# lyd405121/ti-raytrace

Measured on AMD Instinct MI355X. Metric: Mrays/s (primary+secondary) at 1024² 100k-tri, 1/2/4/8 GPU + HBM GB/s, higher is better.
Workload: dtype f32

## Files before the change

ti_raytrace_amd/_native.py:

```python
import ctypes as C
import os

import numpy as np

_HERE = os.path.dirname(os.path.abspath(__file__))
LIB_PATH = os.environ.get("TIRT_LIB_PATH") or os.path.join(_HERE, "csrc", "libtirt.so")

_f32p = np.ctypeslib.ndpointer(dtype=np.float32, flags="C_CONTIGUOUS")
_i32p = np.ctypeslib.ndpointer(dtype=np.int32, flags="C_CONTIGUOUS")


class TirtError(RuntimeError):
    pass


class TirtStackOverflow(TirtError):

    def __init__(self, msg, stats):
        TirtError.__init__(self, msg)
        self.stats = stats


ERR_STACK = -4

# ... 22 lines not shown
DEBUG_GNORMAL = 3

AOV_WORDS = 8
AOV_ALBEDO = 0
AOV_NORMAL = 3
AOV_DEPTH = 6
AOV_ALPHA = 7

MOM_WORDS = 8
MOM_N = 0
MOM_MEAN = 1
MOM_M2 = 4
MOM_BAD = 7

MOTION_WORDS = 8

SF_GLASS, SF_ENV, SF_LIGHT_TRI, SF_LIGHT_SPOT_LASER, SF_NO_LIGHT, SF_LIGHT_SPHERE, SF_LIGHT_OTHER = 1, 2, 4, 8, 16, 32, 64
SF_ALL = 127
SF_TEXTURE = 128
SHADE_INSTANTIATIONS = (SF_LIGHT_SPHERE, SF_LIGHT_TRI, SF_ALL, SF_ALL | SF_TEXTURE)
SF_TEXTURE_PARAM = 256
SHADE_INSTANTIATION_MAPS = SF_ALL | SF_TEXTURE | SF_TEXTURE_PARAM
SF_CUTOUT = 512
SF_ENV_SAMPLE = 1024
SHADE_INSTANTIATIONS_ENV = (SF_ALL | SF_ENV_SAMPLE, SHADE_INSTANTIATION_MAPS | SF_ENV_SAMPLE)
KAT_ENV_SAMPLE_IN, KAT_ENV_SAMPLE_OUT = 2, 10
KAT_ENV_PDF_IN, KAT_ENV_PDF_OUT = 3, 5
KAT_ALPHA_IN, KAT_ALPHA_OUT = 3, 2
KAT_MAPS_IN, KAT_MAPS_OUT = 3, 8
KAT_STEP_IN, KAT_STEP_OUT = 23, 28

OPTIONS = {
    "shade_specialize": (1, "1: the narrowest instantiation of k_shade / k_shade_spec that covers the scene's feature word; 0: the generic kernel"),
}

_vp = C.c_void_p
SIGNATURES = {
    "tirt_last_error": (C.c_char_p, []),
    "tirt_version": (C.c_int, []),
    "tirt_device_count": (C.c_int, [C.POINTER(C.c_int)]),
    "tirt_create": (C.c_int, [C.c_int, C.POINTER(_vp)]),
    "tirt_destroy": (None, [_vp]),
    "tirt_sync": (C.c_int, [_vp]),
    "tirt_set_option": (C.c_int, [_vp, C.c_char_p, C.c_double]),
    "tirt_scene_upload": (C.c_int, [_vp, _f32p, C.c_int, _i32p, C.c_int, _f32p, C.c_int,
                                    _f32p, C.c_int, _i32p, C.c_int, C.c_int, _f32p, _f32p]),
    "tirt_material_upload": (C.c_int, [_vp, _f32p, C.c_int]),
    "tirt_env_upload": (C.c_int, [_vp, _i32p, C.c_int, C.c_int, C.c_float]),
    "tirt_texture_upload": (C.c_int, [_vp, C.c_int, _vp, C.c_int64, _vp, _vp, _vp, _vp]),
    "tirt_kat_texture": (C.c_int, [_vp, _f32p, C.c_int, _f32p, C.c_int, C.c_int]),
    "tirt_kat_material_maps": (C.c_int, [_vp, _f32p, C.c_int, _f32p, C.c_int, C.c_int]),
    "tirt_texture_cutout": (C.c_int, [_vp, _vp, C.c_int]),
    "tirt_kat_texture_alpha": (C.c_int, [_vp, _f32p, C.c_int, _f32p, C.c_int, C.c_int]),
    "tirt_shade_features": (C.c_int, [_vp, C.POINTER(C.c_uint32)]),
    "tirt_shade_features_host": (C.c_int, [_f32p, C.c_int, _i32p, C.c_int, _f32p, C.c_int, _i32p, C.c_int, _vp, C.c_int, C.c_int, C.c_float,
                                           C.POINTER(C.c_uint32)]),
    "tirt_shade_features_host_env": (C.c_int, [_f32p, C.c_int, _i32p, C.c_int, _f32p, C.c_int, _i32p, C.c_int, _vp, C.c_int, C.c_int, C.c_float,
                                               C.c_int, C.POINTER(C.c_uint32)]),
    "tirt_env_sampling": (C.c_int, [_vp, C.c_int, C.c_float]),
    "tirt_env_table_download": (C.c_int, [_vp, _vp, _vp, _vp, C.POINTER(C.c_int32)]),
    "tirt_kat_env_sample": (C.c_int, [_vp, _f32p, C.c_int, _f32p, C.c_int, C.c_int]),
    "tirt_kat_env_pdf": (C.c_int, [_vp, _f32p, C.c_int, _f32p, C.c_int, C.c_int]),
    "tirt_lbvh_build": (C.c_int, [_vp]),
    "tirt_lbvh_download": (C.c_int, [_vp, _vp, _vp, _vp]),
    "tirt_traversal_tree_download": (C.c_int, [_vp, _vp]),
    "tirt_wide_tree_download": (C.c_int, [_vp, _vp, _vp, _vp, _vp, _vp, _vp]),
# ... 733 lines not shown
```

ti_raytrace_amd/csrc/tirt_api.hip:

```cpp
#include "tirt_internal.h"
#include "tirt_spectral.h"
#include <stddef.h>
#include <algorithm>
#include <mutex>
#include <string.h>

namespace tirt {

static thread_local std::string g_error;
void set_error(const std::string &msg) { g_error = msg; }

SceneView scene_view(const tirt_ctx *c)
{
    SceneView s;
    s.vertex = c->vertex.as<float>(); s.primitive = c->primitive.as<int>(); s.material = c->material.as<float>();
    s.shape = c->shape.as<float>(); s.light = c->light.as<int>(); s.env = c->env.as<int>();
    s.mat_lrgb = c->mat_lrgb.as<float>(); s.shade_rec = c->shade_rec.as<float4>(); s.light_rec = c->light_rec.as<float4>();
    s.tex = c->tex_count > 0 ? c->tex.as<int>() : nullptr;
    s.n = c->n; s.light_count = c->light_count; s.env_w = c->env_w; s.env_h = c->env_h; s.env_power = c->env_power;
    return s;
}
BvhView bvh_view(const tirt_ctx *c)
{
    BvhView b;
// ... 452 lines not shown
    if (!strcmp(name, "plan_batches")) { TIRT_REQUIRE(value >= 0.0 && value <= 64.0, "plan_batches: 0 (automatic) .. 64"); if (flush_pending(c)) return TIRT_ERR_HIP; c->plan_nb = (int)value; return TIRT_OK; }
    if (!strcmp(name, "plan_lanes")) { TIRT_REQUIRE(value >= 0.0 && value <= TIRT_MAX_LANES, "plan_lanes: 0 (automatic) .. the lane count"); if (flush_pending(c)) return TIRT_ERR_HIP; c->plan_lanes = (int)value; return TIRT_OK; }
    if (!strcmp(name, "job_frames")) { TIRT_REQUIRE(value >= 0.0 && value <= 1.0e9, "job_frames out of range"); c->job_frames = (long)value; return TIRT_OK; }
    if (!strcmp(name, "merge_paths")) { TIRT_REQUIRE(value >= 0.0 && value <= 1.0e9, "merge_paths out of range"); c->merge_paths = (size_t)value; c->merge_user = true; return TIRT_OK; }
    if (!strcmp(name, "batch_paths")) {
        TIRT_REQUIRE(value >= 1.0 && value <= 1.0e9, "tirt_set_option: batch_paths out of range");
        c->batch_paths = (size_t)value; c->batch_user = true; return TIRT_OK;
    }
    if (!strcmp(name, "trace_lds_depth")) {
        TIRT_REQUIRE(value >= 12 && value <= 64, "trace_lds_depth: 12..64");
        TIRT_REQUIRE(trace_lds_bytes((int)value) <= c->lds_optin, "trace_lds_depth: stacks + tree top exceed the LDS a block can have on this device");
        c->tr_lds_depth = (int)value; return TIRT_OK;
    }
    if (!strcmp(name, "bdpt_stack_size")) { TIRT_REQUIRE(value >= 16 && value <= 4096, "bdpt_stack_size: 16..4096"); c->bdpt_stack = (int)value; return TIRT_OK; }
    if (!strcmp(name, "trace_timeline")) { c->timeline_arm = (int)value; c->timeline_waves = 0; return TIRT_OK; }
    if (!strcmp(name, "trace_refill_min")) { TIRT_REQUIRE(value >= 1 && value <= 64, "trace_refill_min: 1..64"); c->tr_refill_min = (int)value; return TIRT_OK; }
    if (!strcmp(name, "trace_node_min")) { TIRT_REQUIRE(value >= 1 && value <= 64, "trace_node_min: 1..64"); c->tr_node_min = (int)value; return TIRT_OK; }
    if (!strcmp(name, "bdpt_bounded")) { c->bdpt_bounded = value != 0.0 ? 1 : 0; return TIRT_OK; }
    if (!strcmp(name, "bdpt_state_fill")) { TIRT_REQUIRE(value == 0.0 || value == 1.0 || value == 2.0, "bdpt_state_fill: 0 (none), 1 (zeros) or 2 (poison)"); c->bdpt_state_fill = (int)value; return TIRT_OK; }
    if (!strcmp(name, "primary_beams")) { TIRT_REQUIRE(value == 0.0 || value == 1.0, "primary_beams: 0 or 1"); if (flush_pending(c)) return TIRT_ERR_HIP; c->primary_beams = (int)value; return TIRT_OK; }
    if (!strcmp(name, "primary_beams_rebuild")) { if (flush_pending(c)) return TIRT_ERR_HIP; c->pvb_valid = false; return TIRT_OK; }
    if (!strcmp(name, "primary_beams_diag")) { if (flush_pending(c)) return TIRT_ERR_HIP; c->pvb_diag = value != 0.0; return TIRT_OK; }
    if (!strcmp(name, "primary_beams_min_frames")) { TIRT_REQUIRE(value >= 1.0 && value <= 1.0e6, "primary_beams_min_frames out of range"); if (flush_pending(c)) return TIRT_ERR_HIP; c->primary_beams_min_frames = (int)value; return TIRT_OK; }
    if (!strcmp(name, "bdpt_lanes")) { TIRT_REQUIRE(value >= 1.0 && value <= 4.0, "bdpt_lanes: 1..4"); if (sync_all(c)) return TIRT_ERR_HIP; c->bdpt_lanes = (int)value; return TIRT_OK; }
    if (!strcmp(name, "bdpt_batch_items")) { TIRT_REQUIRE(value >= 1.0 && value <= 1.0e9, "bdpt_batch_items out of range"); c->bdpt_batch_items = (size_t)value; return TIRT_OK; }
    if (!strcmp(name, "bdpt_mem_budget")) { TIRT_REQUIRE(value >= 0, "bdpt_mem_budget: bytes >= 0"); c->bdpt_mem_budget = (size_t)value; return TIRT_OK; }
    if (!strcmp(name, "trace_slices")) {
        const int iv = (int)value;
        TIRT_REQUIRE(iv >= 1 && iv <= 64 && (iv & (iv - 1)) == 0, "trace_slices: power of two, 1..64");
        int l = 0; while ((1 << l) < iv) l++;
        c->tr_slice_log2 = l; return TIRT_OK;
    }
    if (!strcmp(name, "shade_specialize")) { TIRT_REQUIRE(value == 0.0 || value == 1.0, "shade_specialize: 0 (generic kernel) or 1"); if (flush_pending(c)) return TIRT_ERR_HIP; c->shade_specialize = (int)value; return TIRT_OK; }
    if (!strcmp(name, "shade_grid")) { TIRT_REQUIRE(value >= 1 && value <= 65536, "shade_grid: 1..65536"); c->sh_grid = (int)value; c->grid_user = true; return TIRT_OK; }
    if (!strcmp(name, "path_order_blocks")) { c->path_order_blocks = value != 0.0; return TIRT_OK; }
    if (!strcmp(name, "slices_contiguous")) { c->slices_contiguous = value != 0.0; return TIRT_OK; }
    if (!strcmp(name, "trace_grid_alone")) { TIRT_REQUIRE(value >= 1 && value <= 16384, "trace_grid_alone: 1..16384"); c->tr_grid_alone = (int)value; return TIRT_OK; }
    if (!strcmp(name, "query_chunk_rays")) {
        TIRT_REQUIRE(value >= 256.0 && value <= (double)(1 << 27), "query_chunk_rays: 256 .. 2^27");
        c->query_chunk = (size_t)value; return TIRT_OK;
    }
    if (!strcmp(name, "trace_grid")) { TIRT_REQUIRE(value >= 1 && value <= 16384, "trace_grid: 1..16384"); c->tr_grid = (int)value; c->grid_user = true; return TIRT_OK; }
    set_error(std::string("tirt_set_option: unknown option ") + name);
    return TIRT_ERR_ARG;
}

int tirt_scene_upload(tirt_ctx *c, const float *vertex, int nv, const int32_t *primitive, int n, const float *material, int nm,
                      const float *shape, int ns, const int32_t *light, int nl, int light_count, const float bmin[3], const float bmax[3])
{
    CTX(c);
    if (sync_all(c)) return TIRT_ERR_HIP;
    TIRT_REQUIRE(n >= 1 && nv >= 0 && nm >= 1 && ns >= 1 && nl >= 1, "tirt_scene_upload: need n,nm,ns,nl >= 1");
    TIRT_REQUIRE(vertex && primitive && material && shape && light && bmin && bmax, "tirt_scene_upload: null pointer");
    TIRT_REQUIRE(light_count >= 0 && light_count <= nl, "tirt_scene_upload: light_count out of range");
    TIRT_REQUIRE((long long)2 * n - 1 < (1ll << 24), "tirt_scene_upload: node indices are stored as f32 (exact below 2^24 nodes)");
    for (int i = 0; i < n; i++) {
        const int32_t *pr = primitive + (size_t)i * 3;
        if (pr[0] == PRIMITIVE_TRI) { TIRT_REQUIRE(pr[1] >= 0 && pr[1] + 2 < nv, "tirt_scene_upload: vertex index out of range"); }
        else { TIRT_REQUIRE(pr[1] >= 0 && pr[1] < ns, "tirt_scene_upload: shape index out of range"); }
        TIRT_REQUIRE(pr[2] >= 0 && pr[2] < nm, "tirt_scene_upload: material index out of range");
    }
    for (int i = 0; i < nl; i++) TIRT_REQUIRE(light[i] >= 0 && light[i] < n, "tirt_scene_upload: light index out of range");
    if (int rc = check_material_textures("tirt_scene_upload", material, nm, c->tex_count)) return rc;
    c->sphere_prims.clear(); c->sphere_geom.clear();
    c->h_mat_on_tri.assign((size_t)nm, 0);
    for (int i = 0; i < n; i++) {
// ... 684 lines not shown
        (void)hipEventRecord(c->ev1, c->stream);
        e = hipEventSynchronize(c->ev1);
        float ms = 0.0f;
        if (e == hipSuccess) e = hipEventElapsedTime(&ms, c->ev0, c->ev1);
        if (rep > 0 && ms < best) best = ms;
    }
    rec.release(); out.release();
    TIRT_HIP(e);
    *gbps_out = (double)blocks * 256.0 * (double)iters * 64.0 / ((double)best * 1.0e-3) / 1.0e9;
    return TIRT_OK;
}

int tirt_stats(tirt_ctx *c, tirt_stats_t *out)
{
    CTX(c);
    TIRT_REQUIRE(out, "tirt_stats: null");
    if (ensure_counters(c)) return TIRT_ERR_HIP;
    DevCounters h;
    if (sync_all(c)) return TIRT_ERR_HIP;
    TIRT_HIP(hipMemcpyAsync(&h, c->dev_counters.p, sizeof(h), hipMemcpyDeviceToHost, c->stream));
    TIRT_HIP(hipStreamSynchronize(c->stream));
    drain_render_events(c);
    out->rays_closest = h.rays_closest; out->rays_shadow = h.rays_shadow;
    out->box_closest = h.box_closest; out->leaf_closest = h.leaf_closest;
    out->box_shadow = h.box_shadow; out->leaf_shadow = h.leaf_shadow;
    out->shaded = h.shaded; out->paths = h.paths; out->stack_overflow = h.stack_overflow;
    out->diag_it_node = h.it_node; out->diag_lanes_node = h.lanes_node; out->diag_it_leaf = h.it_leaf;
    out->diag_lanes_leaf = h.lanes_leaf; out->diag_refills = h.refills; out->diag_it_outer = h.it_outer;
    out->diag_wave_ticks = h.wave_ticks; out->diag_drain_ticks = h.drain_ticks; out->diag_waves = h.waves;
    out->ms_build = c->ms_build; out->ms_render = c->ms_render;
    out->ms_trace_closest = c->ms_trace_closest; out->ms_trace_shadow = c->ms_trace_shadow; out->ms_shade = c->ms_shade;
    out->launches_trace_closest = c->launches_trace_closest; out->launches_trace_shadow = c->launches_trace_shadow;
    out->launches_shade = c->launches_shade; out->launches_tail = 0;
    if (h.stack_overflow > 0) {
        set_error("traversal stack overflow on " + std::to_string((unsigned long long)h.stack_overflow) + " rays: raise stack_size");
        TIRT_HIP(hipMemsetAsync((char *)c->dev_counters.p + offsetof(DevCounters, stack_overflow), 0, sizeof(h.stack_overflow), c->stream));
        TIRT_HIP(hipStreamSynchronize(c->stream));
        return TIRT_ERR_STACK;
    }
    return TIRT_OK;
}

static void drain_pvb_events(tirt_ctx *c)
{
    for (auto &pr : c->pvb_ev) {
        float ms = 0.0f;
        if (hipEventElapsedTime(&ms, pr.first, pr.second) == hipSuccess) c->pvb_build_ns += (unsigned long long)((double)ms * 1.0e6);
        (void)hipEventDestroy(pr.first); (void)hipEventDestroy(pr.second);
    }
    c->pvb_ev.clear();
    (void)hipGetLastError();
}

int tirt_primary_beam_stats(tirt_ctx *c, uint64_t out[12])
{
    TIRT_REQUIRE(c && out, "tirt_primary_beam_stats: null arguments");
    for (int k = 0; k < 12; k++) out[k] = 0;
    if (sync_all(c)) return TIRT_ERR_HIP;
    drain_pvb_events(c);
    out[5] = c->pvb_builds; out[6] = c->pvb_build_ns; out[7] = c->pvb_skipped;
    if (!c->pvb_stat.p) return TIRT_OK;
    unsigned long long h[12];
    TIRT_HIP(hipMemcpy(h, c->pvb_stat.p, sizeof(h), hipMemcpyDeviceToHost));
    for (int k = 0; k < 5; k++) out[k] = h[k];
    for (int k = 8; k < 12; k++) out[k] = h[k];
    return TIRT_OK;
// ... 43 lines not shown
```

ti_raytrace_amd/csrc/tirt_internal.h:

```cpp
#pragma once
#include <hip/hip_runtime.h>
#include <stdint.h>
#include <stdio.h>
#include <initializer_list>
#include <string>
#include <type_traits>
#include <vector>
#include "../../include/tirt.h"
#include "tirt_device.h"

namespace tirt {

void set_error(const std::string &msg);

#define TIRT_HIP(call)                                                                          \
    do {                                                                                        \
        hipError_t e__ = (call);                                                                \
        if (e__ != hipSuccess) {                                                                \
            tirt::set_error(std::string(#call) + ": " + hipGetErrorString(e__));                \
            return TIRT_ERR_HIP;                                                                \
        }                                                                                       \
    } while (0)

#define TIRT_REQUIRE(cond, msg)                                                                 \
// ... 139 lines not shown
    float *sdist;
    int *sdst;
    float *fr, *fg, *fb;
    float *scw, *fw;
};

struct TileMap { int tile_rank, tile_count, tile_size, H, blocked, F; const int *pixels; };
TD void slot_to_frame_pixel(const TileMap &m, int P, int slot, int &f, int &k)
{
    if (m.F > 0) { const int c = slot >> 6, kb = c / m.F; f = c - kb * m.F; k = (kb << 6) | (slot & 63); }
    else { f = slot / P; k = slot - f * P; }
}
TD int frame_pixel_to_slot(const TileMap &m, int P, int f, int k)
{ return m.F > 0 ? ((((k >> 6) * m.F + f) << 6) | (k & 63)) : f * P + k; }
TD int local_to_pixel(const TileMap &m, int k)
{
    int lt = k / m.tile_size, within = k - lt * m.tile_size;
    if (m.blocked) {
        const int rows = m.H >> 3;
        const int b = within >> 6, l = within & 63;
        const int bc = b / rows, bj = b - bc * rows;
        within = ((bc << 3) + (l >> 3)) * m.H + (bj << 3) + (l & 7);
    }
    return (lt * m.tile_count + m.tile_rank) * m.tile_size + within;
}

template <bool LIST> TD int mapped_pixel(const TileMap &m, int k) { if constexpr (LIST) return m.pixels[k]; else return local_to_pixel(m, k); }

struct DevCounters {
    unsigned long long rays_closest, rays_shadow, box_closest, leaf_closest, box_shadow, leaf_shadow;
    unsigned long long shaded, paths, stack_overflow;
    unsigned long long it_node, lanes_node, it_leaf, lanes_leaf, refills, it_outer;
    unsigned long long wave_ticks, drain_ticks, waves;
};

#define TIRT_MAX_LANES 8
struct Lane {
    hipStream_t stream = nullptr;
    hipEvent_t film_done = nullptr; bool film_recorded = false;
    hipEvent_t aov_done = nullptr;
    size_t path_capacity = 0;
    DevBuf path_mem, counters_mem, spill;
    PathState ps;
};

}

struct tirt_ctx {
    int device = 0;
    hipStream_t stream = nullptr;
    hipEvent_t ev0 = nullptr, ev1 = nullptr;

    int nv = 0, n = 0, nm = 0, ns = 0, nl = 0, light_count = 0;
    float bmin[3] = {0, 0, 0}, bmax[3] = {0, 0, 0};
    tirt::DevBuf vertex, primitive, material, shape, light, env, mat_lrgb, shade_rec, light_rec;
    bool shade_rec_valid = false;
    bool light_rec_valid = false;
    int env_w = 0, env_h = 0; float env_power = 0.0f;
    std::vector<int> tex_cutout; std::vector<unsigned char> h_mat_on_tri; bool has_cutout = false;
    tirt::DevBuf cut_uv, cut_flags; bool cut_rec_valid = false, cut_tagged = false;
    tirt::DevBuf tex; int tex_count = 0;
    std::vector<float> h_material; std::vector<int> h_light_kind; bool env_lit = false;
    unsigned shade_features = 127u;
    int env_sample_on = 0; float env_share = 0.5f; bool env_tab_valid = false;
    int shade_specialize = 1;

    bool built = false;
    tirt::DevBuf morton_unsorted;
    tirt::DevBuf keys_a, keys_b, vals_a, vals_b;
    tirt::DevBuf hist;
    tirt::DevBuf morton_sorted;
    tirt::DevBuf bvh_node, compact;
    tirt::DevBuf parent, flag, subtree, build_status, leaf_compact;
    tirt::DevBuf wnode, tri, prim_slot;
    tirt::DevBuf cnode, cparent, csize, wide_queue, wide_levels;
    int wide_nodes = 0;
    tirt::DevBuf sah_compact, sah_csize, sah_parent, wide_dp, sah_box, sah_idx, sah_tasks, sah_counts;
    int use_sah = 1, sah_levels = 0, built_sah = 0;
    std::vector<int> sphere_prims;
    std::vector<float> sphere_geom;
    tirt::DevBuf timeline; int timeline_arm = -1, timeline_waves = 0;
    int n_far_nodes = 0;
    int wide_dp_on = 0;
    float grid_min[3] = {0, 0, 0}, grid_cell[3] = {1, 1, 1}, grid_inv_cell[3] = {1, 1, 1}, grid_inv_extent[3] = {1, 1, 1};
    size_t lds_optin = 65536;
    float root_min[3], root_max[3]; int root_code = 0;
    float wide_pad = 0.0f; int shapes_boxed = 0;

    tirt::CameraView cam; float view[16]; bool cam_set = false;

    int W = 0, H = 0, tile_rank = 0, tile_count = 1, tile_size = 4096, tile_blocked = 0;
    long npix_local = 0;
    tirt::DevBuf hdr, rgb;
    tirt::DevBuf aov;
    hipEvent_t last_aov = nullptr;
    tirt::DevBuf mom, mom_cnt;
    tirt::DevBuf pixset, pixset_tmp; long pixset_n = -1;
    tirt::DevBuf tp_mem; int tp_cur = 0; bool tp_valid = false; tirt_temporal_camera_t tp_cam = {};
// ... 193 lines not shown
```

ti_raytrace_amd/csrc/tirt_render.hip:

```cpp
#include "tirt_internal.h"
#include "tirt_spectral.h"

namespace tirt {

constexpr int TR_GRID_MAX = 2048;

enum { KIND_CLOSEST = 0, KIND_SHADOW_ACC = 1, KIND_MIXED = 2, KIND_QUERY = 3 };
#if !defined(TIRT_EXPERIMENTS) && (defined(TR_PAD) || defined(TR_PADG))
#error "the bound ladder (TR_PAD / TR_PADG) needs an experiments build: add -DTIRT_EXPERIMENTS"
#endif
struct TraceArgs {
    BvhView bvh;
    const float *ox, *oy, *oz, *dx, *dy, *dz;
    float eye[3];
    const int *count_ptr; int count_fixed;
    float4 *hit;
    const int *sprim, *sdst; const float *sdist, *scr, *scg, *scb; float *rr, *rg, *rb, *fr, *fg, *fb;
    const float *scw; float *rw, *fw;
    int *spill; int spill_depth;
    const float *sox, *soy, *soz, *sdx, *sdy, *sdz; const int *scount_ptr;
    int *fetch; int slice_log2;
    int slices_contig;
    int lds_depth;
    int refill_min;
    int node_min;
    DevCounters *ctr; int2 *per_ray_counts;
    unsigned long long *timeline;
    int no_ray_count;
    const float4 *ray4;
    const int *ray_index;
};
struct TraceArgsCut : TraceArgs { CutView cut; };
template <bool CUTOUT> struct trace_args_of { typedef TraceArgs type; };
template <> struct trace_args_of<true> { typedef TraceArgsCut type; };

struct ShadeStep {
    bool want_next = false, want_shadow = false, shaded = false;
    v3 next_o = V(0.0f, 0.0f, 0.0f), next_d = next_o, next_thr = next_o, sh_o = next_o, sh_d = next_o, sh_c = next_o;
    float next_pdf = 0.0f, sh_dist = 0.0f; int next_spec = 0, sh_expect = -2;
};
template <unsigned FEAT, bool LIST = false>
TD void shade_path(const SceneView &sc, const TileMap &tm, int P, uint32_t frame_begin, uint32_t seed, int bounce, int last_bounce, int slot,
                   const v3 origin, const v3 direction, const float4 hrec, v3 throughout, v3 &radiance, float brdf_pdf, int perfect_spec, ShadeStep &s)
{
    int f, k; slot_to_frame_pixel(tm, P, slot, f, k);
    const uint32_t pixel = (uint32_t)mapped_pixel<LIST>(tm, k);
    const uint32_t frame = frame_begin + (uint32_t)f;
    const uint32_t dim0 = TM_DIM_BOUNCE0 + TM_DIMS_PER_BOUNCE * (uint32_t)bounce;
    const float t = hrec.x;
    constexpr bool ENV_NEE = (FEAT & SF_ENV_SAMPLE) != 0u;
    [[maybe_unused]] float p_env = 0.0f;
    if constexpr (ENV_NEE) p_env = sc.light_count == 0 ? 1.0f : env_table(sc).share;
    if (t < INF_VALUE) {
        const int prim_id = __float_as_int(hrec.w);
        int mat_id;
        const HitAttr h = hit_attributes_rec<(FEAT & (SF_TEXTURE | SF_TEXTURE_PARAM)) != 0u>(sc.shade_rec, origin, direction, prim_id, t, hrec.y, hrec.z, mat_id);
        v3 normal = h.nor;
        if constexpr ((FEAT & SF_TEXTURE_PARAM) != 0u) {
            const int nor_id = material_map(sc.material + (size_t)mat_id * MAT_VEC, 9);
            if (nor_id >= 0) normal = tex_normal_rec(sc.tex, sc.shade_rec, nor_id, prim_id, h.tex, normal);
        }
        const v3 fnormal = normal * signf(dot(-direction, h.gnor));
        const float *m = sc.material + (size_t)mat_id * MAT_VEC;
        const v3 mat_color = V(m[2], m[3], m[4]);
// ... 519 lines not shown
        }

        const bool from_pend = STASH && pend != 0;
        const bool leaf_now = have && (from_pend || (cur < 0 && cur != TR_SENT));
        if (COUNT) {
            const int n_l = __popcll(ballot64(leaf_now));
            if (n_l) { d_it_leaf++; d_lanes_leaf += (unsigned long long)n_l; }
        }
        if (leaf_now) {
            const int code = ~(from_pend ? pend : cur);
            if (COUNT) nleaf += 1;
            bool accepted;
            if constexpr (CUTOUT) accepted = trace_leaf_step<MODE != TIRT_TRAVERSE_EXHAUSTIVE, true, CutSource>(b, r, par, code, hit_t, hit_u, hit_v, hit_prim, hit_leaf);
            else accepted = trace_leaf_step<MODE != TIRT_TRAVERSE_EXHAUSTIVE>(b, r, par, code, hit_t, hit_u, hit_v, hit_prim, hit_leaf);
            if (from_pend) pend = 0; else TR_POP(cur);
            if (accepted) {
                lim = __builtin_fminf(__builtin_fminf(cull_far < 0.0f ? INF_VALUE : hit_t * 1.0001f, __builtin_fabsf(cull_far)), INF_VALUE);
                if (BOUNDED && hit_prim != expect && hit_t < settle) { cur = TR_SENT; paged = 0; pend = 0; }
            }
        }

        if (ballot64(have && cur == TR_SENT && paged > 0) != 0ull) {
            if (have && cur == TR_SENT && paged > 0) { TR_PAGE_IN(); TR_POP(cur); }
        }

        if (have && cur == TR_SENT && pend == 0) {
            TR_COLD(ca);
            float4 *const c_hit = ca->hit;
            const int *const c_sdst = MAY_SHADOW ? ca->sdst : nullptr;
            float *const c_rr = MAY_SHADOW ? ca->rr : nullptr, *const c_rg = MAY_SHADOW ? ca->rg : nullptr, *const c_rb = MAY_SHADOW ? ca->rb : nullptr;
            float *const c_fr = MAY_SHADOW ? ca->fr : nullptr, *const c_fg = MAY_SHADOW ? ca->fg : nullptr, *const c_fb = MAY_SHADOW ? ca->fb : nullptr;
            const float *const c_scr = MAY_SHADOW ? ca->scr : nullptr, *const c_scg = MAY_SHADOW ? ca->scg : nullptr, *const c_scb = MAY_SHADOW ? ca->scb : nullptr;
            const float *const c_scw = MAY_SHADOW ? ca->scw : nullptr;
            if (MAY_SHADOW) asm volatile("" :: "s"(c_hit), "s"(c_sdst), "s"(c_rr), "s"(c_rg), "s"(c_rb), "s"(c_fr), "s"(c_fg), "s"(c_fb), "s"(c_scr), "s"(c_scg), "s"(c_scb), "s"(c_scw));
            if (!(MAY_SHADOW && is_sh) || KIND == KIND_QUERY) {
                { typedef float f4n __attribute__((ext_vector_type(4))); f4n hv__ = {hit_t, hit_u, hit_v, __int_as_float(hit_prim)}; __builtin_nontemporal_store(hv__, (f4n *)&c_hit[q]); }
            } else if (hit_prim == expect) {
                const int dst = TR_LDS_(c_sdst[q]);
                float *pr = dst >= 0 ? c_rr + dst : c_fr + ~dst;
                float *pg = dst >= 0 ? c_rg + dst : c_fg + ~dst;
                float *pb = dst >= 0 ? c_rb + dst : c_fb + ~dst;
                *pr = *pr + TR_LDS_(c_scr[q]); *pg = *pg + TR_LDS_(c_scg[q]); *pb = *pb + TR_LDS_(c_scb[q]);
                if (c_scw) { float *pw = dst >= 0 ? ca->rw + dst : ca->fw + ~dst; *pw = *pw + c_scw[q]; }
            }
            if (COUNT) {
                if (MAY_SHADOW && is_sh) { sum_box_s += nbox; sum_leaf_s += nleaf; }
                else { sum_box += nbox; sum_leaf += nleaf; }
                if (ca->per_ray_counts) ca->per_ray_counts[q] = make_int2((int)nbox, (int)nleaf);
            }
            if (n_overflow) n_over++;
            have = false; sa = sa_bottom;
        }
    }
    TR_COLD(ca);
    if (ca->ctr) {
        if (COUNT) {
            sum_box = wave_sum(sum_box); sum_leaf = wave_sum(sum_leaf);
            sum_box_s = wave_sum(sum_box_s); sum_leaf_s = wave_sum(sum_leaf_s);
            if (lane == 0 && (sum_box | sum_leaf)) { atomicAdd(&ca->ctr->box_closest, sum_box); atomicAdd(&ca->ctr->leaf_closest, sum_leaf); }
            if (lane == 0 && (sum_box_s | sum_leaf_s)) { atomicAdd(&ca->ctr->box_shadow, sum_box_s); atomicAdd(&ca->ctr->leaf_shadow, sum_leaf_s); }
        }
        if (COUNT) { d_outer = wave_sum(d_outer); if (lane == 0) atomicAdd(&ca->ctr->it_outer, d_outer); }
        if (COUNT && lane == 0) {
            atomicAdd(&ca->ctr->it_node, d_it_node); atomicAdd(&ca->ctr->lanes_node, d_lanes_node);
            atomicAdd(&ca->ctr->it_leaf, d_it_leaf); atomicAdd(&ca->ctr->lanes_leaf, d_lanes_leaf);
            atomicAdd(&ca->ctr->refills, d_refills);
            const unsigned long long tk_end = wall_clock64();
            atomicAdd(&ca->ctr->wave_ticks, tk_end - tk_start); atomicAdd(&ca->ctr->drain_ticks, tk_end - (tk_exh ? tk_exh : tk_end)); atomicAdd(&ca->ctr->waves, 1ull);
            if (ca->timeline) {
                const unsigned hw = __builtin_amdgcn_s_getreg((31 << 11) | 4), xcc = __builtin_amdgcn_s_getreg((31 << 11) | 20);
                unsigned long long *rec = ca->timeline + (size_t)(gtid >> 6) * 4;
                rec[0] = tk_start; rec[1] = tk_exh; rec[2] = tk_end; rec[3] = (unsigned long long)hw | ((unsigned long long)xcc << 32);
            }
        }
        if (n_over) atomicAdd(&ca->ctr->stack_overflow, n_over);
        if (gtid == 0 && !ca->no_ray_count) {
// ... 522 lines not shown
    TIRT_REQUIRE(!(feat & (SF_TEXTURE | SF_TEXTURE_PARAM)) || c->tex_count > 0, "tirt_kat_shade_step: the textured instantiation needs uploaded textures (tirt_texture_upload): without them no material row's slot is checked");
    for (int i = 0; i < n; i++) {
        const float *a = in + (size_t)i * in_stride;
        const int32_t *w = (const int32_t *)a; const int32_t prim = w[14], pixel = w[1];
        TIRT_REQUIRE(!(a[11] < INF_VALUE) || (prim >= 0 && prim < c->n), "tirt_kat_shade_step: row " + std::to_string(i) + ": prim outside [0, n_prims) of a hit (t < INF)");
        TIRT_REQUIRE(pixel >= 0 && pixel < 0x7fffffff, "tirt_kat_shade_step: row " + std::to_string(i) + ": pixel outside [0, 2^31 - 1)");
    }
    if (n == 0) return TIRT_OK;
    if (sync_all(c)) return TIRT_ERR_HIP;
    if (ensure_shade_records(c)) return TIRT_ERR_HIP;
    return kat_round_trip(c, "tirt_kat_shade_step", {{in, kat_row_bytes(n, in_stride)}}, out, kat_row_bytes(n, out_stride), [&](const void *const *din, void *dout) {
        hipLaunchKernelGGL(fn, dim3((n + SH_BLOCK - 1) / SH_BLOCK), dim3(SH_BLOCK), 0, c->stream, scene_view(c), (const float *)din[0], in_stride, (float *)dout, out_stride, n);
    });
}

__global__ void k_film_spec(PathState ps, const float *fw, SpecView sp, TileMap tm, int P, int F, uint32_t frame_begin, uint32_t seed, float *hdr)
{
    int k = blockIdx.x * blockDim.x + threadIdx.x;
    if (k >= P) return;
    const int p = local_to_pixel(tm, k);
    float *px = hdr + (size_t)p * 3;
    float r = px[0], g = px[1], b = px[2];
    for (int f = 0; f < F; f++) {
        const int s = frame_pixel_to_slot(tm, P, f, k);
        const uint32_t frame = frame_begin + (uint32_t)f;
        const float coff = 1.0f / ((float)(int)frame + 1.0f);
        const float Lambda = HERO_LAMBDA_MIN + HERO_LAMBDA_STEP * tm_rand(seed, (uint32_t)p, frame, TM_DIM_SPEC_LAMBDA);
        f4s spec; spec.v[0] = ps.fr[s]; spec.v[1] = ps.fg[s]; spec.v[2] = ps.fb[s]; spec.v[3] = fw[s];
        spec_add_splat(sp, spec, Lambda, coff, r, g, b);
    }
    px[0] = r; px[1] = g; px[2] = b;
}

constexpr size_t LINE = 128;
static size_t lane_counter_bytes(int max_depth)
{ return LINE * (size_t)(max_depth + 1) + sizeof(int) * TR_FETCH_STRIDE * TR_FETCH_LINES * (size_t)(max_depth + 1); }

constexpr int PATH_WORDS = 2 * 15 + 4 + 12 + 3 + 2;
static size_t path_state_bytes(size_t S) { return sizeof(float) * PATH_WORDS * ((S + 3) & ~(size_t)3); }
static int ensure_paths(Lane &L, size_t S, int max_depth)
{
    if (S > L.path_capacity || !L.path_mem.p) {
        if (L.path_mem.ensure(path_state_bytes(S))) return TIRT_ERR_HIP;
        const size_t S_user = S;
        S = (S + 3) & ~(size_t)3;
        float *w = L.path_mem.as<float>();
        PathState &p = L.ps;
        auto nxt = [&]() { float *r = w; w += S; return r; };
        for (int k = 0; k < 2; k++) {
            PathSoA &q = p.st[k];
            q.ox = nxt(); q.oy = nxt(); q.oz = nxt(); q.dx = nxt(); q.dy = nxt(); q.dz = nxt();
            q.tr = nxt(); q.tg = nxt(); q.tb = nxt(); q.rr = nxt(); q.rg = nxt(); q.rb = nxt();
            q.brdf_pdf = nxt(); q.flags = (uint32_t *)nxt(); q.slot = (int *)nxt();
        }
        p.hit = (float4 *)w; w += 4 * S;
        p.sox = nxt(); p.soy = nxt(); p.soz = nxt(); p.sdx = nxt(); p.sdy = nxt(); p.sdz = nxt();
        p.scr = nxt(); p.scg = nxt(); p.scb = nxt(); p.sprim = (int *)nxt(); p.sdist = nxt(); p.sdst = (int *)nxt();
        p.fr = nxt(); p.fg = nxt(); p.fb = nxt();
        p.scw = nxt(); p.fw = nxt();
        L.path_capacity = S_user;
    }
    if (L.counters_mem.ensure(lane_counter_bytes(max_depth))) return TIRT_ERR_HIP;
    return 0;
}

int pt_render(tirt_ctx *c, uint32_t frame_begin, int frame_count, uint32_t seed, int max_depth, int stack_size, int flags, const SpecView *spec)
// ... 71 lines not shown
            if (begin) { hipEvent_t a, b; (void)hipEventCreate(&a); (void)hipEventCreate(&b); v.push_back({a, b}); (void)hipEventRecord(a, st); }
            else (void)hipEventRecord(v.back().second, st);
        };

        TIRT_HIP(hipMemsetAsync(L.counters_mem.p, 0, lane_counter_bytes(max_depth), st));
        hipLaunchKernelGGL(list ? k_generate<true> : k_generate<false>, dim3((S + B - 1) / B), dim3(B), 0, st, L.ps.st[0], c->cam, tm, P, S, f0, seed, ctr);
        bool busy = false;
        if (c->last_film) { busy = hipEventQuery(c->last_film) == hipErrorNotReady; (void)hipGetLastError(); }
        const BatchPlan plan = plan_batches(c);
        const bool two_big = plan.lanes <= 2 && plan.batch >= ((size_t)24 << 20) && !c->grid_user;
        const int grid_cap = (busy && n_lanes > 1 && !two_big) ? c->tr_grid : c->tr_grid_alone;
        int grid_full = (S + TR_BLOCK - 1) / TR_BLOCK; if (grid_full > grid_cap) grid_full = grid_cap;
        const int sh_cap = two_big ? 2 * c->sh_grid : c->sh_grid;
        int grid_shade = (S + SH_BLOCK - 1) / SH_BLOCK; if (grid_shade > sh_cap) grid_shade = sh_cap;
        v3 eye_v; eye_v.x = c->cam.eye[0]; eye_v.y = c->cam.eye[1]; eye_v.z = c->cam.eye[2];
        const shade_fn_t shade_fn = list ? pick_shade_rgb(c).fn_list : pick_shade_rgb(c).fn;
        const shade_spec_fn_t shade_spec_fn = pick_shade_inst(SHADE_SPEC_INST, c).fn;
        for (int b = 0; b < max_depth; b++) {
            const PathSoA &in = L.ps.st[b & 1], &out = L.ps.st[(b + 1) & 1];
            TraceArgs a = {};
            a.bvh = bv;
            a.ox = in.ox; a.oy = in.oy; a.oz = in.oz; a.dx = in.dx; a.dy = in.dy; a.dz = in.dz;
            if (b == 0) { a.ox = a.oy = a.oz = nullptr; for (int k = 0; k < 3; k++) a.eye[k] = c->cam.eye[k]; }
            a.count_ptr = (b == 0) ? nullptr : cnt_path(b); a.count_fixed = S;
            a.hit = L.ps.hit;
            a.spill = L.spill.as<int>(); a.spill_depth = spill_depth; a.ctr = ctr; a.per_ray_counts = nullptr;
            a.fetch = fetch(b);
            a.sox = L.ps.sox; a.soy = L.ps.soy; a.soz = L.ps.soz; a.sdx = L.ps.sdx; a.sdy = L.ps.sdy; a.sdz = L.ps.sdz;
            a.sprim = L.ps.sprim; a.sdst = L.ps.sdst; a.sdist = L.ps.sdist; a.scr = L.ps.scr; a.scg = L.ps.scg; a.scb = L.ps.scb;
            a.rr = in.rr; a.rg = in.rg; a.rb = in.rb; a.fr = L.ps.fr; a.fg = L.ps.fg; a.fb = L.ps.fb;
            if (spec) { a.scw = L.ps.scw; a.rw = (float *)in.flags; a.fw = L.ps.fw; }
            a.scount_ptr = (b == 0) ? nullptr : cnt_shadow(b - 1);
            fill_tunables(c, a);
            a.timeline = timeline_for(c, flags, grid_full);
            if (!(b == 0 && use_beams)) stamp(evc, true);
            if (b == 0 && use_beams) {
                int *const fb_count = (int *)append_ctr(0) + 4;
                float4 *const fb_hit = (float4 *)L.ps.sox;
                pvb_launch_cand(c, st, bv, in.dx, in.dy, in.dz, tm, P, S, L.ps.hit, fb_count, (int *)out.ox, out.dx, out.dy, out.dz, ctr);
                TraceArgs a2 = a;
                a2.dx = out.dx; a2.dy = out.dy; a2.dz = out.dz; a2.count_ptr = fb_count; a2.count_fixed = S; a2.hit = fb_hit; a2.no_ray_count = 1;
                stamp(evc, true);
                if (int rc = launch_trace<KIND_CLOSEST>(c, st, a2, flags, grid_full)) return rc;
                stamp(evc, false);
                pvb_launch_scatter(st, fb_count, (const int *)out.ox, fb_hit, L.ps.hit);
            } else
            if (int rc = (b == 0) ? launch_trace<KIND_CLOSEST>(c, st, a, flags, grid_full) : launch_trace<KIND_MIXED>(c, st, a, flags, grid_full)) return rc;
            if (!(b == 0 && use_beams)) stamp(evc, false);
            c->launches_trace_closest++;
            if (b == 0 && c->aov.p) { if (int rc = aov_launch(c, L, tm, P, F, f0)) return rc; }

            stamp(evh, true);
            if (spec)
                hipLaunchKernelGGL(shade_spec_fn, dim3(grid_shade), dim3(SH_BLOCK), 0, st, ShadeArgs{L.ps, in, out}, sv, *spec, tm, P, f0, seed, b,
                                   (b == max_depth - 1) ? 1 : 0, (b == 0) ? (const int *)nullptr : cnt_path(b), S,
                                   append_ctr(b), ctr, eye_v);
            else
            hipLaunchKernelGGL(shade_fn, dim3(grid_shade), dim3(SH_BLOCK), 0, st, ShadeArgs{L.ps, in, out}, sv, tm, P, f0, seed, b,
                               (b == max_depth - 1) ? 1 : 0, (b == 0) ? (const int *)nullptr : cnt_path(b), S,
                               append_ctr(b), ctr, eye_v);
            stamp(evh, false);
            c->launches_shade++;

            if (b == max_depth - 1) {
                TraceArgs sa = {};
                sa.bvh = bv;
                sa.ox = L.ps.sox; sa.oy = L.ps.soy; sa.oz = L.ps.soz; sa.dx = L.ps.sdx; sa.dy = L.ps.sdy; sa.dz = L.ps.sdz;
                sa.count_ptr = cnt_shadow(b); sa.count_fixed = 0;
                sa.sprim = L.ps.sprim; sa.sdst = L.ps.sdst; sa.sdist = L.ps.sdist; sa.scr = L.ps.scr; sa.scg = L.ps.scg; sa.scb = L.ps.scb;
                sa.rr = out.rr; sa.rg = out.rg; sa.rb = out.rb; sa.fr = L.ps.fr; sa.fg = L.ps.fg; sa.fb = L.ps.fb;
                if (spec) { sa.scw = L.ps.scw; sa.rw = (float *)out.flags; sa.fw = L.ps.fw; }
                sa.spill = L.spill.as<int>(); sa.spill_depth = spill_depth; sa.ctr = ctr; sa.per_ray_counts = nullptr;
                sa.fetch = fetch(max_depth);
                fill_tunables(c, sa);
                stamp(evs, true);
                if (int rc = launch_trace<KIND_SHADOW_ACC>(c, st, sa, flags, grid_full)) return rc;
                stamp(evs, false);
                c->launches_trace_shadow++;
            }
        }
        if (c->last_film) TIRT_HIP(hipStreamWaitEvent(st, c->last_film, 0));
        if (spec) hipLaunchKernelGGL(k_film_spec, dim3((P + B - 1) / B), dim3(B), 0, st, L.ps, L.ps.fw, *spec, tm, P, F, f0, seed, c->hdr.as<float>());
        else hipLaunchKernelGGL(list ? k_film<true> : k_film<false>, dim3((P + B - 1) / B), dim3(B), 0, st, L.ps, tm, P, F, f0, c->hdr.as<float>());
        if (c->mom.p && !spec) { if (int rc = moments_launch(c, L, tm, P, F)) return rc; }
        TIRT_HIP(hipEventRecord(L.film_done, st));
        L.film_recorded = true;
        c->last_film = L.film_done;
        if (use_beams) c->pvb_set[c->pvb_cur].busy = L.film_done;
        TIRT_HIP(hipEventRecord(r1, st));
        if (c->time_kernels) {
            TIRT_HIP(hipStreamSynchronize(st));
            auto drain = [&](std::vector<std::pair<hipEvent_t, hipEvent_t>> &v, double &acc) {
                for (auto &pr : v) { float ms = 0; (void)hipEventElapsedTime(&ms, pr.first, pr.second); acc += ms; (void)hipEventDestroy(pr.first); (void)hipEventDestroy(pr.second); }
                v.clear();
            };
            drain(evc, c->ms_trace_closest); drain(evs, c->ms_trace_shadow); drain(evh, c->ms_shade);
        }
        c->ev_pool.push_back({r0, r1});
        if (c->ev_pool.size() > 64) {
            size_t keep = 0;
            for (auto &pr : c->ev_pool) {
                if (hipEventQuery(pr.second) == hipSuccess) {
                    float ms = 0.0f;
                    if (hipEventElapsedTime(&ms, pr.first, pr.second) == hipSuccess) c->ms_render += ms;
                    (void)hipEventDestroy(pr.first); (void)hipEventDestroy(pr.second);
                } else c->ev_pool[keep++] = pr;
            }
            c->ev_pool.resize(keep);
            (void)hipGetLastError();
// ... 8 lines not shown
```

Baseline: 5687.

## Defer shadow-ray contribution accumulation to a dense k_shadow_apply pass

Shadow rays in k_trace now write a hit/miss verdict into the sprim buffer instead of doing scattered read-modify-write accumulation into radiance buffers at write-back. A new k_shadow_apply kernel then walks the shadow queue densely and adds the contributions for unoccluded rays. The aim is to take the divergent scattered gathers and stores out of the traversal kernel's tail, which should lighten its register and memory pressure. The cost is an extra kernel launch per bounce and a second pass over the shadow arrays.

New measurement: 5725 (median of 6 runs). About the same (+0.7%).

```diff
diff --git a/ti_raytrace_amd/_native.py b/ti_raytrace_amd/_native.py
--- a/ti_raytrace_amd/_native.py
+++ b/ti_raytrace_amd/_native.py
@@ -78,6 +78,7 @@
 
 OPTIONS = {
     "shade_specialize": (1, "1: the narrowest instantiation of k_shade / k_shade_spec that covers the scene's feature word; 0: the generic kernel"),
+    "shadow_apply": (1, "1: k_trace's shadow rays store a verdict and k_shadow_apply adds their contributions in a dense pass; 0: k_trace adds them at write-back"),
 }
 
 _vp = C.c_void_p
diff --git a/ti_raytrace_amd/csrc/tirt_api.hip b/ti_raytrace_amd/csrc/tirt_api.hip
--- a/ti_raytrace_amd/csrc/tirt_api.hip
+++ b/ti_raytrace_amd/csrc/tirt_api.hip
@@ -508,6 +508,7 @@
         c->tr_slice_log2 = l; return TIRT_OK;
     }
     if (!strcmp(name, "shade_specialize")) { TIRT_REQUIRE(value == 0.0 || value == 1.0, "shade_specialize: 0 (generic kernel) or 1"); if (flush_pending(c)) return TIRT_ERR_HIP; c->shade_specialize = (int)value; return TIRT_OK; }
+    if (!strcmp(name, "shadow_apply")) { TIRT_REQUIRE(value == 0.0 || value == 1.0, "shadow_apply: 0 (k_trace adds at write-back) or 1 (verdict + k_shadow_apply)"); if (flush_pending(c)) return TIRT_ERR_HIP; c->shadow_apply = (int)value; return TIRT_OK; }
     if (!strcmp(name, "shade_grid")) { TIRT_REQUIRE(value >= 1 && value <= 65536, "shade_grid: 1..65536"); c->sh_grid = (int)value; c->grid_user = true; return TIRT_OK; }
     if (!strcmp(name, "path_order_blocks")) { c->path_order_blocks = value != 0.0; return TIRT_OK; }
     if (!strcmp(name, "slices_contiguous")) { c->slices_contiguous = value != 0.0; return TIRT_OK; }
@@ -1258,6 +1259,9 @@
     out->ms_trace_closest = c->ms_trace_closest; out->ms_trace_shadow = c->ms_trace_shadow; out->ms_shade = c->ms_shade;
     out->launches_trace_closest = c->launches_trace_closest; out->launches_trace_shadow = c->launches_trace_shadow;
     out->launches_shade = c->launches_shade; out->launches_tail = 0;
+#ifdef TIRT_SHADOW_ARRIVE_COUNT
+    out->launches_tail = h.shadow_arrived;
+#endif
     if (h.stack_overflow > 0) {
         set_error("traversal stack overflow on " + std::to_string((unsigned long long)h.stack_overflow) + " rays: raise stack_size");
         TIRT_HIP(hipMemsetAsync((char *)c->dev_counters.p + offsetof(DevCounters, stack_overflow), 0, sizeof(h.stack_overflow), c->stream));
diff --git a/ti_raytrace_amd/csrc/tirt_internal.h b/ti_raytrace_amd/csrc/tirt_internal.h
--- a/ti_raytrace_amd/csrc/tirt_internal.h
+++ b/ti_raytrace_amd/csrc/tirt_internal.h
@@ -195,6 +195,9 @@
     unsigned long long shaded, paths, stack_overflow;
     unsigned long long it_node, lanes_node, it_leaf, lanes_leaf, refills, it_outer;
     unsigned long long wave_ticks, drain_ticks, waves;
+#ifdef TIRT_SHADOW_ARRIVE_COUNT
+    unsigned long long shadow_arrived;
+#endif
 };
 
 #define TIRT_MAX_LANES 8
@@ -227,6 +230,7 @@
     unsigned shade_features = 127u;
     int env_sample_on = 0; float env_share = 0.5f; bool env_tab_valid = false;
     int shade_specialize = 1;
+    int shadow_apply = 1;
 
     bool built = false;
     tirt::DevBuf morton_unsorted;
diff --git a/ti_raytrace_amd/csrc/tirt_render.hip b/ti_raytrace_amd/csrc/tirt_render.hip
--- a/ti_raytrace_amd/csrc/tirt_render.hip
+++ b/ti_raytrace_amd/csrc/tirt_render.hip
@@ -24,12 +24,14 @@
     int lds_depth;
     int refill_min;
     int node_min;
+    int shadow_apply;
     DevCounters *ctr; int2 *per_ray_counts;
     unsigned long long *timeline;
     int no_ray_count;
     const float4 *ray4;
     const int *ray_index;
 };
+static_assert(offsetof(TraceArgs, ctr) - offsetof(TraceArgs, fetch) == 32, "TraceArgs::shadow_apply fills the padding between node_min and ctr");
 struct TraceArgsCut : TraceArgs { CutView cut; };
 template <bool CUTOUT> struct trace_args_of { typedef TraceArgs type; };
 template <> struct trace_args_of<true> { typedef TraceArgsCut type; };
@@ -615,16 +617,30 @@
             float *const c_fr = MAY_SHADOW ? ca->fr : nullptr, *const c_fg = MAY_SHADOW ? ca->fg : nullptr, *const c_fb = MAY_SHADOW ? ca->fb : nullptr;
             const float *const c_scr = MAY_SHADOW ? ca->scr : nullptr, *const c_scg = MAY_SHADOW ? ca->scg : nullptr, *const c_scb = MAY_SHADOW ? ca->scb : nullptr;
             const float *const c_scw = MAY_SHADOW ? ca->scw : nullptr;
+            constexpr bool ACCUMULATES = MAY_SHADOW && KIND != KIND_QUERY;
+            float *const c_rw = ACCUMULATES ? ca->rw : nullptr, *const c_fw = ACCUMULATES ? ca->fw : nullptr;
+            int *const c_verdict = (ACCUMULATES && ca->shadow_apply) ? const_cast<int *>(ca->sprim) : nullptr;
             if (MAY_SHADOW) asm volatile("" :: "s"(c_hit), "s"(c_sdst), "s"(c_rr), "s"(c_rg), "s"(c_rb), "s"(c_fr), "s"(c_fg), "s"(c_fb), "s"(c_scr), "s"(c_scg), "s"(c_scb), "s"(c_scw));
+            if (ACCUMULATES) asm volatile("" :: "s"(c_rw), "s"(c_fw), "s"(c_verdict));
             if (!(MAY_SHADOW && is_sh) || KIND == KIND_QUERY) {
                 { typedef float f4n __attribute__((ext_vector_type(4))); f4n hv__ = {hit_t, hit_u, hit_v, __int_as_float(hit_prim)}; __builtin_nontemporal_store(hv__, (f4n *)&c_hit[q]); }
+            } else if (c_verdict) {
+                __builtin_nontemporal_store((int)(hit_prim == expect), &c_verdict[q]);
+            } else if (c_scw) {
+                if (hit_prim == expect) {
+                    const int dst = TR_LDS_(c_sdst[q]);
+                    const float cr = TR_LDS_(c_scr[q]), cg = TR_LDS_(c_scg[q]), cb = TR_LDS_(c_scb[q]), cw = c_scw[q];
+                    float *const pr = dst >= 0 ? c_rr + dst : c_fr + ~dst, *const pg = dst >= 0 ? c_rg + dst : c_fg + ~dst;
+                    float *const pb = dst >= 0 ? c_rb + dst : c_fb + ~dst, *const pw = dst >= 0 ? c_rw + dst : c_fw + ~dst;
+                    const float vr = *pr, vg = *pg, vb = *pb, vw = *pw;
+                    *pr = vr + cr; *pg = vg + cg; *pb = vb + cb; *pw = vw + cw;
+                }
             } else if (hit_prim == expect) {
                 const int dst = TR_LDS_(c_sdst[q]);
-                float *pr = dst >= 0 ? c_rr + dst : c_fr + ~dst;
-                float *pg = dst >= 0 ? c_rg + dst : c_fg + ~dst;
-                float *pb = dst >= 0 ? c_rb + dst : c_fb + ~dst;
-                *pr = *pr + TR_LDS_(c_scr[q]); *pg = *pg + TR_LDS_(c_scg[q]); *pb = *pb + TR_LDS_(c_scb[q]);
-                if (c_scw) { float *pw = dst >= 0 ? ca->rw + dst : ca->fw + ~dst; *pw = *pw + c_scw[q]; }
+                const float cr = TR_LDS_(c_scr[q]), cg = TR_LDS_(c_scg[q]), cb = TR_LDS_(c_scb[q]);
+                float *const pr = dst >= 0 ? c_rr + dst : c_fr + ~dst, *const pg = dst >= 0 ? c_rg + dst : c_fg + ~dst, *const pb = dst >= 0 ? c_rb + dst : c_fb + ~dst;
+                const float vr = *pr, vg = *pg, vb = *pb;
+                *pr = vr + cr; *pg = vg + cg; *pb = vb + cb;
             }
             if (COUNT) {
                 if (MAY_SHADOW && is_sh) { sum_box_s += nbox; sum_leaf_s += nleaf; }
@@ -1213,6 +1229,37 @@
     px[0] = r; px[1] = g; px[2] = b;
 }
 
+__global__ __launch_bounds__(256) void k_shadow_apply(PathState ps, float *rr, float *rg, float *rb, float *rw, float *fw, const float *scw, const int *count_ptr, DevCounters *ctr)
+{
+    const int n = *count_ptr;
+    const int stride = (int)gridDim.x * 256;
+#ifdef TIRT_SHADOW_ARRIVE_COUNT
+    unsigned long long arrived = 0;
+#endif
+    for (int qs = (int)blockIdx.x * 256 + (int)threadIdx.x; qs < n; qs += stride) {
+        if (__builtin_nontemporal_load(&ps.sprim[qs]) == 0) continue;
+        const int dst = __builtin_nontemporal_load(&ps.sdst[qs]);
+        const float cr = __builtin_nontemporal_load(&ps.scr[qs]), cg = __builtin_nontemporal_load(&ps.scg[qs]), cb = __builtin_nontemporal_load(&ps.scb[qs]);
+        float *const pr = dst >= 0 ? rr + dst : ps.fr + ~dst, *const pg = dst >= 0 ? rg + dst : ps.fg + ~dst, *const pb = dst >= 0 ? rb + dst : ps.fb + ~dst;
+        const float vr = *pr, vg = *pg, vb = *pb;
+        *pr = vr + cr; *pg = vg + cg; *pb = vb + cb;
+        if (scw) { float *const pw = dst >= 0 ? rw + dst : fw + ~dst; *pw = *pw + scw[qs]; }
+#ifdef TIRT_SHADOW_ARRIVE_COUNT
+        arrived++;
+#endif
+    }
+#ifdef TIRT_SHADOW_ARRIVE_COUNT
+    arrived = wave_sum(arrived);
+    if ((threadIdx.x & 63) == 0 && arrived) atomicAdd(&ctr->shadow_arrived, arrived);
+#endif
+}
+constexpr int SA_GRID_MAX = 4096;
+static void shadow_apply_launch(hipStream_t st, int S, const PathState &ps, float *rr, float *rg, float *rb, float *rw, bool spec, const int *count_ptr, DevCounters *ctr)
+{
+    int grid = (S + 255) / 256; if (grid > SA_GRID_MAX) grid = SA_GRID_MAX; if (grid < 1) grid = 1;
+    hipLaunchKernelGGL(k_shadow_apply, dim3(grid), dim3(256), 0, st, ps, rr, rg, rb, spec ? rw : nullptr, spec ? ps.fw : nullptr, spec ? ps.scw : (const float *)nullptr, count_ptr, ctr);
+}
+
 constexpr size_t LINE = 128;
 static size_t lane_counter_bytes(int max_depth)
 { return LINE * (size_t)(max_depth + 1) + sizeof(int) * TR_FETCH_STRIDE * TR_FETCH_LINES * (size_t)(max_depth + 1); }
@@ -1350,6 +1397,7 @@
             if (spec) { a.scw = L.ps.scw; a.rw = (float *)in.flags; a.fw = L.ps.fw; }
             a.scount_ptr = (b == 0) ? nullptr : cnt_shadow(b - 1);
             fill_tunables(c, a);
+            a.shadow_apply = c->shadow_apply;
             a.timeline = timeline_for(c, flags, grid_full);
             if (!(b == 0 && use_beams)) stamp(evc, true);
             if (b == 0 && use_beams) {
@@ -1366,6 +1414,11 @@
             if (int rc = (b == 0) ? launch_trace<KIND_CLOSEST>(c, st, a, flags, grid_full) : launch_trace<KIND_MIXED>(c, st, a, flags, grid_full)) return rc;
             if (!(b == 0 && use_beams)) stamp(evc, false);
             c->launches_trace_closest++;
+            if (b > 0 && c->shadow_apply) {
+                stamp(evs, true);
+                shadow_apply_launch(st, S, L.ps, in.rr, in.rg, in.rb, (float *)in.flags, spec != nullptr, cnt_shadow(b - 1), ctr);
+                stamp(evs, false);
+            }
             if (b == 0 && c->aov.p) { if (int rc = aov_launch(c, L, tm, P, F, f0)) return rc; }
 
             stamp(evh, true);
@@ -1391,8 +1444,10 @@
                 sa.spill = L.spill.as<int>(); sa.spill_depth = spill_depth; sa.ctr = ctr; sa.per_ray_counts = nullptr;
                 sa.fetch = fetch(max_depth);
                 fill_tunables(c, sa);
+                sa.shadow_apply = c->shadow_apply;
                 stamp(evs, true);
                 if (int rc = launch_trace<KIND_SHADOW_ACC>(c, st, sa, flags, grid_full)) return rc;
+                if (c->shadow_apply) shadow_apply_launch(st, S, L.ps, out.rr, out.rg, out.rb, (float *)out.flags, spec != nullptr, cnt_shadow(b), ctr);
                 stamp(evs, false);
                 c->launches_trace_shadow++;
             }
```
